# rbuler/multimodal-isic

Measured on AMD Instinct MI355X. Metric: bags/sec (train step) @ 64x224x224 patches/bag, higher is better.
Workload: dtype bf16; 1 GPU; ISIC-shaped attention-MIL: 256 bags x 64x224x224 patches + 128-d radiomics, ResNet-18 encoder, bf16 (BASELINE.json configs[1]); patches_per_bag=64, patch=3x224x224, radiomics_dim=128, parallelism=dp1

## Files before the change

### multimodal-isic_amd/csrc/conv_stem.hip

```cpp
#include <type_traits>

#include "common.h"
#include "slab_sum.inc"
#include "mfma_tile.h"
#include "pool_grad.h"

namespace {

constexpr int TH = 8, TW = 16;
constexpr int PR = 2 * TH + 5, PC = 40;
constexpr int PROW = PC * 8;
constexpr int WROW = 7 * 64 + 16;
constexpr int CPAD = 72;
constexpr int YROW = 128 + 32;
constexpr int STEM_DW_ELEMS = 64 * 7 * 7 * 3;
constexpr int STEM_WGRAD_BLOCKS = 512;
constexpr int STEM_FWD_BLOCKS = 768;

struct StemArgs {
  const unsigned short* in;
  const unsigned short* w;
  unsigned short* out;
  const unsigned short* dy;
  float* dw;
  double* stat_sum;
  double* stat_sumsq;
  int stat_slots;
  int N, Hin, Win, Hout, Wout, tiles_h, tiles_w, total_tiles;
};

constexpr int PATCH_PER_THREAD = (PR * PC + 255) / 256;
__device__ __forceinline__ void fetch_patch(u32x2 (&r)[PATCH_PER_THREAD], const StemArgs& a, int tile, int tid) {
  const int n = tile / (a.tiles_h * a.tiles_w);
  const int t2 = tile - n * (a.tiles_h * a.tiles_w);
  const int oy0 = (t2 / a.tiles_w) * TH, ox0 = (t2 % a.tiles_w) * TW;
#pragma unroll
  for (int u = 0; u < PATCH_PER_THREAD; ++u) {
    const int idx = tid + 256 * u;
    const int pr = idx / PC, pc = idx - pr * PC;
    const int hi = 2 * oy0 - 3 + pr, wi = 2 * ox0 - 3 + pc;
    u32x2 v = {0u, 0u};
    if (tile < a.total_tiles && idx < PR * PC && hi >= 0 && hi < a.Hin && wi >= 0 && wi < a.Win)
      v = *reinterpret_cast<const u32x2*>(a.in + (((size_t)n * a.Hin + hi) * a.Win + wi) * 4);
    r[u] = v;
  }
}
__device__ __forceinline__ void commit_patch(unsigned char* Ps, const u32x2 (&r)[PATCH_PER_THREAD], int tid) {
#pragma unroll
  for (int u = 0; u < PATCH_PER_THREAD; ++u) {
    const int idx = tid + 256 * u;
    if (idx < PR * PC) {
      const int pr = idx / PC, pc = idx - pr * PC;
      *reinterpret_cast<u32x2*>(Ps + pr * PROW + pc * 8) = r[u];
    }
  }
}

__global__ __launch_bounds__(256) void conv_stem_fwd_kernel(StemArgs a) {
  static_assert(TH * TW * CPAD * 2 >= PR * PROW, "the C tile overlays the patch");
  __shared__ __attribute__((aligned(16))) unsigned char smem[64 * WROW + TH * TW * CPAD * 2];
  unsigned char* Ws = smem;
  unsigned char* Ps = smem + 64 * WROW;
  unsigned short* Cs = reinterpret_cast<unsigned short*>(smem + 64 * WROW);
  const int tid = threadIdx.x, lane = tid & 63, wave = tid >> 6;
  const int fi = lane & 15, fg = lane >> 4;

  for (int idx = tid; idx < 64 * 28; idx += 256) {
    const int co = idx / 28, ch = idx - co * 28;
    *reinterpret_cast<u32x4*>(Ws + co * WROW + ch * 16) = *reinterpret_cast<const u32x4*>(a.w + co * 224 + ch * 8);
  }

  u32x2 pre[PATCH_PER_THREAD];
  fetch_patch(pre, a, blockIdx.x, tid);
  float st_s[4][4], st_q[4][4];
#pragma unroll
  for (int j = 0; j < 4; ++j)
#pragma unroll
    for (int r = 0; r < 4; ++r) { st_s[j][r] = 0.f; st_q[j][r] = 0.f; }
  for (int tile = blockIdx.x; tile < a.total_tiles; tile += gridDim.x) {
    const int n = tile / (a.tiles_h * a.tiles_w);
    const int t2 = tile - n * (a.tiles_h * a.tiles_w);
    const int oy0 = (t2 / a.tiles_w) * TH, ox0 = (t2 % a.tiles_w) * TW;
    lds_barrier();
    commit_patch(Ps, pre, tid);
    lds_barrier();
    fetch_patch(pre, a, tile + gridDim.x, tid);

    f32x4 acc[2][4];
#pragma unroll
    for (int i = 0; i < 2; ++i)
#pragma unroll
      for (int j = 0; j < 4; ++j) acc[i][j] = (f32x4){0.f, 0.f, 0.f, 0.f};
#pragma unroll
    for (int kh = 0; kh < 7; ++kh) {
      bf16x8 af[2], bfr[4];
#pragma unroll
      for (int i = 0; i < 2; ++i) {
        const int oyl = wave * 2 + i;
        af[i] = *reinterpret_cast<const bf16x8*>(Ps + (2 * oyl + kh) * PROW + (2 * fi + 2 * fg) * 8);
      }
#pragma unroll
      for (int j = 0; j < 4; ++j)
        bfr[j] = *reinterpret_cast<const bf16x8*>(Ws + (j * 16 + fi) * WROW + kh * 64 + fg * 16);
#pragma unroll
      for (int i = 0; i < 2; ++i)
#pragma unroll
        for (int j = 0; j < 4; ++j)
          acc[i][j] = __builtin_amdgcn_mfma_f32_16x16x32_bf16(bfr[j], af[i], acc[i][j], 0, 0, 0);
    }
    lds_barrier();
#pragma unroll
    for (int i = 0; i < 2; ++i)
#pragma unroll
      for (int j = 0; j < 4; ++j) {
        const int p = (wave * 2 + i) * 16 + fi;
        const u32x2 v = isic_pack_bf16x4(acc[i][j]);
        *reinterpret_cast<u32x2*>(Cs + p * CPAD + j * 16 + fg * 4) = v;
        if (a.stat_sum) {
          const bool in = (oy0 + wave * 2 + i < a.Hout) && (ox0 + fi < a.Wout);
          const float r0 = in ? __uint_as_float(v[0] << 16) : 0.f, r1 = in ? __uint_as_float(v[0] & 0xFFFF0000u) : 0.f;
          const float r2 = in ? __uint_as_float(v[1] << 16) : 0.f, r3 = in ? __uint_as_float(v[1] & 0xFFFF0000u) : 0.f;
          st_s[j][0] += r0; st_q[j][0] += r0 * r0;
          st_s[j][1] += r1; st_q[j][1] += r1 * r1;
          st_s[j][2] += r2; st_q[j][2] += r2 * r2;
          st_s[j][3] += r3; st_q[j][3] += r3 * r3;
        }
      }
    lds_barrier();
    for (int idx = tid; idx < TH * TW * 8; idx += 256) {
      const int p = idx >> 3, ch = idx & 7;
      const int oy = oy0 + (p >> 4), ox = ox0 + (p & 15);
      if (oy < a.Hout && ox < a.Wout)
        __builtin_nontemporal_store(*reinterpret_cast<const u32x4*>(Cs + p * CPAD + ch * 8),
                                    reinterpret_cast<u32x4*>(a.out + (((size_t)n * a.Hout + oy) * a.Wout + ox) * 64 + ch * 8));
    }
  }
  if (a.stat_sum) {
    __shared__ float stat_red[2][4][64];
    lds_barrier();
#pragma unroll
    for (int j = 0; j < 4; ++j)
#pragma unroll
      for (int r = 0; r < 4; ++r) {
        float sv = st_s[j][r], qv = st_q[j][r];
#pragma unroll
        for (int o = 8; o > 0; o >>= 1) { sv += __shfl_xor(sv, o, 16); qv += __shfl_xor(qv, o, 16); }
        if (fi == 0) { stat_red[0][wave][j * 16 + fg * 4 + r] = sv; stat_red[1][wave][j * 16 + fg * 4 + r] = qv; }
      }
    lds_barrier();
    if (tid < 128) {
      const int c = tid & 63, w = tid >> 6;
      const float t = (stat_red[w][0][c] + stat_red[w][1][c]) + (stat_red[w][2][c] + stat_red[w][3][c]);
      const size_t slot = (size_t)(blockIdx.x % a.stat_slots) * 64 + c;
      atomicAdd((w == 0 ? a.stat_sum : a.stat_sumsq) + slot, (double)t);
    }
  }
}

__global__ __launch_bounds__(256) void conv_stem_wgrad_kernel(StemArgs a) {
  __shared__ __attribute__((aligned(16))) unsigned char smem[PR * PROW + TH * TW * YROW];
  unsigned char* Ps = smem;
  unsigned char* Ys = smem + PR * PROW;
  const int tid = threadIdx.x, lane = tid & 63, wave = tid >> 6;
  const int fg = lane >> 4, fi = lane & 15, fq = fi >> 2, fp = fi & 3;
  typedef __attribute__((address_space(3))) s16x4* lds_s16x4;

  f32x4 acc[4][4];
#pragma unroll
  for (int i = 0; i < 4; ++i)
#pragma unroll
    for (int j = 0; j < 4; ++j) acc[i][j] = (f32x4){0.f, 0.f, 0.f, 0.f};

  u32x2 pre[PATCH_PER_THREAD];
  u32x4 prey[4];
  auto fetch_dy = [&](int tile) {
    const int n = tile / (a.tiles_h * a.tiles_w);
    const int t2 = tile - n * (a.tiles_h * a.tiles_w);
    const int oy0 = (t2 / a.tiles_w) * TH, ox0 = (t2 % a.tiles_w) * TW;
#pragma unroll
    for (int u = 0; u < 4; ++u) {
      const int idx = tid + 256 * u;
      const int p = idx >> 3, ch = idx & 7;
      const int oy = oy0 + (p >> 4), ox = ox0 + (p & 15);
      u32x4 v = {0u, 0u, 0u, 0u};
      if (tile < a.total_tiles && oy < a.Hout && ox < a.Wout)
        v = *reinterpret_cast<const u32x4*>(a.dy + (((size_t)n * a.Hout + oy) * a.Wout + ox) * 64 + ch * 8);
      prey[u] = v;
    }
  };
  fetch_patch(pre, a, blockIdx.x, tid);
  fetch_dy(blockIdx.x);
  for (int tile = blockIdx.x; tile < a.total_tiles; tile += gridDim.x) {
    lds_barrier();
    commit_patch(Ps, pre, tid);
#pragma unroll
    for (int u = 0; u < 4; ++u) {
      const int idx = tid + 256 * u;
      *reinterpret_cast<u32x4*>(Ys + (idx >> 3) * YROW + (idx & 7) * 16) = prey[u];
    }
    lds_barrier();
    fetch_patch(pre, a, tile + gridDim.x, tid);
    fetch_dy(tile + gridDim.x);
#pragma unroll
    for (int ks = 0; ks < 4; ++ks) {
      const int k1 = ks * 32 + 8 * fg + fq, k2 = k1 + 4;
      bf16x8 af[4], bfr[4];
#pragma unroll
      for (int i = 0; i < 4; ++i) {
        const s16x4 lo = __builtin_amdgcn_ds_read_tr16_b64_v4i16((lds_s16x4)(Ys + k1 * YROW + (i * 16 + 4 * fp) * 2));
        const s16x4 hi = __builtin_amdgcn_ds_read_tr16_b64_v4i16((lds_s16x4)(Ys + k2 * YROW + (i * 16 + 4 * fp) * 2));
        s16x8_t t; t.lo = lo; t.hi = hi;
        af[i] = __builtin_bit_cast(bf16x8, t);
      }
#pragma unroll
      for (int j = 0; j < 4; ++j) {
        const int nt = wave + 4 * j;
        const int kh = nt >> 1, half = nt & 1;
        const int khc = kh > 6 ? 6 : kh;
        const unsigned char* p1 = Ps + (2 * (k1 >> 4) + khc) * PROW + (2 * (k1 & 15) + half * 4 + fp) * 8;
        const unsigned char* p2 = Ps + (2 * (k2 >> 4) + khc) * PROW + (2 * (k2 & 15) + half * 4 + fp) * 8;
        const s16x4 lo = __builtin_amdgcn_ds_read_tr16_b64_v4i16((lds_s16x4)p1);
        const s16x4 hi = __builtin_amdgcn_ds_read_tr16_b64_v4i16((lds_s16x4)p2);
        s16x8_t t; t.lo = lo; t.hi = hi;
        bfr[j] = __builtin_bit_cast(bf16x8, t);
      }
#pragma unroll
      for (int i = 0; i < 4; ++i)
#pragma unroll
        for (int j = 0; j < 4; ++j)
          acc[i][j] = __builtin_amdgcn_mfma_f32_16x16x32_bf16(af[i], bfr[j], acc[i][j], 0, 0, 0);
    }
  }
#pragma unroll
  for (int i = 0; i < 4; ++i)
#pragma unroll
    for (int j = 0; j < 4; ++j) {
      const int nt = wave + 4 * j;
      if (nt >= 14) continue;
      const int kh = nt >> 1, kw = (nt & 1) * 4 + (fi >> 2), c = fi & 3;
      if (kw >= 7 || c >= 3) continue;
#pragma unroll
      for (int r = 0; r < 4; ++r) {
        const int co = i * 16 + fg * 4 + r;
        a.dw[(size_t)blockIdx.x * STEM_DW_ELEMS + ((co * 7 + kh) * 7 + kw) * 3 + c] = acc[i][j][r];
      }
    }
}

struct StemBnArgs {
  StemArgs s;
  const unsigned short* y0;
  const unsigned char* argmax;
  const unsigned short* gp;
  const float* mean; const float* rstd; const float* gamma; const float* scale; const float* shift;
  const double* dgamma; const double* dbeta;
  float* dgamma_f32; float* dbeta_f32;
  int Hp, Wp;
};

__global__ __launch_bounds__(256, 2) void conv_stem_wgrad_bn_kernel(StemBnArgs b) {
  const StemArgs& a = b.s;
  __shared__ __attribute__((aligned(16))) unsigned char smem[PR * PROW + TH * TW * YROW];
  __shared__ __attribute__((aligned(16))) float cst[5][64];
  unsigned char* Ps = smem;
  unsigned char* Ys = smem + PR * PROW;
  const int tid = threadIdx.x, lane = tid & 63, wave = tid >> 6;
  const int fg = lane >> 4, fi = lane & 15, fq = fi >> 2, fp = fi & 3;
  typedef __attribute__((address_space(3))) s16x4* lds_s16x4;
  const isic_pool::PoolGeom geom{a.Hout, a.Wout, 64, b.Hp, b.Wp};

  if (tid < 64) {
    const float inv_rows = 1.f / (float)((int64_t)a.N * a.Hout * a.Wout);
    const float rs = b.rstd[tid], mu = b.mean[tid], k1 = b.gamma[tid] * rs;
    const float k2 = (float)b.dbeta[tid] * inv_rows, k3 = (float)b.dgamma[tid] * inv_rows;
    cst[0][tid] = k1; cst[1][tid] = -k1 * k3 * rs; cst[2][tid] = k1 * (k3 * rs * mu - k2);
    cst[3][tid] = b.scale[tid]; cst[4][tid] = b.shift[tid];
    if (blockIdx.x == 0 && b.dgamma_f32) {
      b.dgamma_f32[tid] += (float)b.dgamma[tid];
      b.dbeta_f32[tid] += (float)b.dbeta[tid];
    }
  }

  f32x4 acc[4][4];
#pragma unroll
  for (int i = 0; i < 4; ++i)
#pragma unroll
    for (int j = 0; j < 4; ++j) acc[i][j] = (f32x4){0.f, 0.f, 0.f, 0.f};

  const int cg = tid & 7, bl = tid >> 3, al = bl >> 3, bw = bl & 7;
  u32x2 pre[PATCH_PER_THREAD];
  u32x4 xr[4];
  isic_pool::Windows win;
  auto fetch_dy = [&](int tile) {
    const int tc = tile < a.total_tiles ? tile : a.total_tiles - 1;
    const int n = tc / (a.tiles_h * a.tiles_w);
    const int t2 = tc - n * (a.tiles_h * a.tiles_w);
    const int oy0 = (t2 / a.tiles_w) * TH, ox0 = (t2 % a.tiles_w) * TW;
    const int ga = (oy0 >> 1) + al, gb = (ox0 >> 1) + bw;
#pragma unroll
    for (int p = 0; p < 4; ++p) {
      const int hi = min(2 * ga + (p >> 1), a.Hout - 1), wi = min(2 * gb + (p & 1), a.Wout - 1);
      xr[p] = *reinterpret_cast<const u32x4*>(b.y0 + (((size_t)n * a.Hout + hi) * a.Wout + wi) * 64 + cg * 8);
    }
    isic_pool::load_windows(win, b.argmax, b.gp, geom, n, min(ga, b.Hp - 1), min(gb, b.Wp - 1), cg);
  };
  auto commit_dy = [&](int tile) {
    const int n = tile / (a.tiles_h * a.tiles_w);
    const int t2 = tile - n * (a.tiles_h * a.tiles_w);
    const int oy0 = (t2 / a.tiles_w) * TH, ox0 = (t2 % a.tiles_w) * TW;
    const int ga = (oy0 >> 1) + al, gb = (ox0 >> 1) + bw;
    const bool inside = (oy0 + TH <= a.Hout) && (ox0 + TW <= a.Wout);
    auto half = [&](auto HC) {
      constexpr int H_ = decltype(HC)::value;
      float g[4][4];
      isic_pool::windows_to_grad4<H_>(win, geom, ga, gb, g);
      const int c0 = cg * 8 + H_ * 4;
      const f32x4 kA = *reinterpret_cast<const f32x4*>(&cst[0][c0]), kB = *reinterpret_cast<const f32x4*>(&cst[1][c0]);
      const f32x4 kD = *reinterpret_cast<const f32x4*>(&cst[2][c0]), sc = *reinterpret_cast<const f32x4*>(&cst[3][c0]);
      const f32x4 sh = *reinterpret_cast<const f32x4*>(&cst[4][c0]);
#pragma unroll
      for (int p = 0; p < 4; ++p) {
        const int oyl = 2 * al + (p >> 1), oxl = 2 * bw + (p & 1);
        const bool in = inside || ((oy0 + oyl < a.Hout) && (ox0 + oxl < a.Wout));
        const unsigned lo = xr[p][2 * H_], hi = xr[p][2 * H_ + 1];
        float xv[4];
        isic_unpack_bf16x4(lo, hi, xv);
        f32x4 o;
#pragma unroll
        for (int j = 0; j < 4; ++j) {
          const float dz = (xv[j] * sc[j] + sh[j] > 0.f) ? g[p][j] : 0.f;
          o[j] = kA[j] * dz + (kB[j] * xv[j] + kD[j]);
          if (!inside) o[j] = in ? o[j] : 0.f;
        }
        *reinterpret_cast<u32x2*>(Ys + (oyl * TW + oxl) * YROW + cg * 16 + H_ * 8) = isic_pack_bf16x4(o);
      }
    };
    half(std::integral_constant<int, 0>{});
    __builtin_amdgcn_sched_barrier(0);
    half(std::integral_constant<int, 1>{});
  };
  __syncthreads();
  fetch_patch(pre, a, blockIdx.x, tid);
  fetch_dy(blockIdx.x);
  for (int tile = blockIdx.x; tile < a.total_tiles; tile += gridDim.x) {
    lds_barrier();
    commit_patch(Ps, pre, tid);
    commit_dy(tile);
    lds_barrier();
    fetch_patch(pre, a, tile + gridDim.x, tid);
    fetch_dy(tile + gridDim.x);
#pragma unroll
    for (int ks = 0; ks < 4; ++ks) {
      const int k1 = ks * 32 + 8 * fg + fq, k2 = k1 + 4;
      bf16x8 af[4], bfr[4];
#pragma unroll
      for (int i = 0; i < 4; ++i) {
        const s16x4 lo = __builtin_amdgcn_ds_read_tr16_b64_v4i16((lds_s16x4)(Ys + k1 * YROW + (i * 16 + 4 * fp) * 2));
        const s16x4 hi = __builtin_amdgcn_ds_read_tr16_b64_v4i16((lds_s16x4)(Ys + k2 * YROW + (i * 16 + 4 * fp) * 2));
        s16x8_t t; t.lo = lo; t.hi = hi;
        af[i] = __builtin_bit_cast(bf16x8, t);
      }
#pragma unroll
      for (int j = 0; j < 4; ++j) {
        const int nt = wave + 4 * j;
        const int kh = nt >> 1, half = nt & 1;
        const int khc = kh > 6 ? 6 : kh;
        const unsigned char* p1 = Ps + (2 * (k1 >> 4) + khc) * PROW + (2 * (k1 & 15) + half * 4 + fp) * 8;
        const unsigned char* p2 = Ps + (2 * (k2 >> 4) + khc) * PROW + (2 * (k2 & 15) + half * 4 + fp) * 8;
        const s16x4 lo = __builtin_amdgcn_ds_read_tr16_b64_v4i16((lds_s16x4)p1);
        const s16x4 hi = __builtin_amdgcn_ds_read_tr16_b64_v4i16((lds_s16x4)p2);
        s16x8_t t; t.lo = lo; t.hi = hi;
        bfr[j] = __builtin_bit_cast(bf16x8, t);
      }
#pragma unroll
      for (int i = 0; i < 4; ++i)
#pragma unroll
        for (int j = 0; j < 4; ++j)
          acc[i][j] = __builtin_amdgcn_mfma_f32_16x16x32_bf16(af[i], bfr[j], acc[i][j], 0, 0, 0);
    }
  }
#pragma unroll
  for (int i = 0; i < 4; ++i)
#pragma unroll
    for (int j = 0; j < 4; ++j) {
      const int nt = wave + 4 * j;
      if (nt >= 14) continue;
      const int kh = nt >> 1, kw = (nt & 1) * 4 + (fi >> 2), c = fi & 3;
      if (kw >= 7 || c >= 3) continue;
#pragma unroll
      for (int r = 0; r < 4; ++r) {
        const int co = i * 16 + fg * 4 + r;
        a.dw[(size_t)blockIdx.x * STEM_DW_ELEMS + ((co * 7 + kh) * 7 + kw) * 3 + c] = acc[i][j][r];
      }
    }
}

__global__ void stem_pack_kernel(const float* __restrict__ w, unsigned short* __restrict__ ws) {
  const int idx = blockIdx.x * blockDim.x + threadIdx.x;
  if (idx >= 64 * 7 * 8 * 4) return;
  const int c = idx & 3, kw = (idx >> 2) & 7, kh = (idx >> 5) % 7, co = idx / 224;
  float v = 0.f;
  if (c < 3 && kw < 7) v = w[((co * 7 + kh) * 7 + kw) * 3 + c];
  ws[idx] = f32_to_bf16_bits(v);
}

int stem_args(StemArgs& a, int N, int Hin, int Win, int Hout, int Wout) {
  if (Hout != (Hin + 6 - 7) / 2 + 1 || Wout != (Win + 6 - 7) / 2 + 1) return ISIC_ERR_BAD_ARG;
  a.N = N; a.Hin = Hin; a.Win = Win; a.Hout = Hout; a.Wout = Wout;
  a.tiles_h = ceil_div(Hout, TH); a.tiles_w = ceil_div(Wout, TW);
  const int64_t tt = (int64_t)N * a.tiles_h * a.tiles_w;
  if (tt > 0x7FFFFFFFLL) return ISIC_ERR_UNSUPPORTED;
  a.total_tiles = (int)tt;
  return ISIC_OK;
}

}

extern "C" {

int isic_conv_stem_fwd_bf16(const uint16_t* in_nhwc4, const uint16_t* w_stem, uint16_t* out, int N, int Hin, int Win,
                            int Hout, int Wout, void* stream) {
  return isic_conv_stem_fwd_stats_bf16(in_nhwc4, w_stem, out, N, Hin, Win, Hout, Wout, nullptr, nullptr, 0, stream);
}

int isic_conv_stem_fwd_stats_bf16(const uint16_t* in_nhwc4, const uint16_t* w_stem, uint16_t* out, int N, int Hin,
                                  int Win, int Hout, int Wout, double* stat_sum, double* stat_sumsq, int stat_slots,
                                  void* stream) {
  ISIC_CHECK_ARG(in_nhwc4 && w_stem && out && N > 0 && Hin > 0 && Win > 0);
  ISIC_CHECK_ARG((stat_sum == nullptr) == (stat_sumsq == nullptr));
  ISIC_CHECK_ARG(!stat_sum || stat_slots > 0);
  StemArgs a;
  a.stat_sum = stat_sum; a.stat_sumsq = stat_sumsq; a.stat_slots = stat_slots > 0 ? stat_slots : 1;
  a.in = in_nhwc4; a.w = w_stem; a.out = out; a.dy = nullptr; a.dw = nullptr;
  int rc = stem_args(a, N, Hin, Win, Hout, Wout);
  if (rc != ISIC_OK) return rc;
  const int grid = a.total_tiles < STEM_FWD_BLOCKS ? a.total_tiles : STEM_FWD_BLOCKS;
  hipLaunchKernelGGL(conv_stem_fwd_kernel, dim3(grid), dim3(256), 0, as_stream(stream), a);
  return isic_launch_status();
}

size_t isic_conv_stem_wgrad_workspace_bytes(void) { return (size_t)STEM_WGRAD_BLOCKS * STEM_DW_ELEMS * sizeof(float); }

int isic_conv_stem_wgrad_bf16(const uint16_t* in_nhwc4, const uint16_t* dy, float* dw, int N, int Hin, int Win,
                              int Hout, int Wout, void* workspace, size_t workspace_bytes, void* stream) {
  ISIC_CHECK_ARG(in_nhwc4 && dy && dw && workspace && N > 0 && Hin > 0 && Win > 0);
  if (workspace_bytes < isic_conv_stem_wgrad_workspace_bytes()) return ISIC_ERR_WORKSPACE;
  StemArgs a;
  a.stat_sum = nullptr; a.stat_sumsq = nullptr; a.stat_slots = 1;
  a.in = in_nhwc4; a.w = nullptr; a.out = nullptr; a.dy = dy; a.dw = reinterpret_cast<float*>(workspace);
  int rc = stem_args(a, N, Hin, Win, Hout, Wout);
  if (rc != ISIC_OK) return rc;
  const int grid = a.total_tiles < STEM_WGRAD_BLOCKS ? a.total_tiles : STEM_WGRAD_BLOCKS;
  hipLaunchKernelGGL(conv_stem_wgrad_kernel, dim3(grid), dim3(256), 0, as_stream(stream), a);
  isic_slab_reduce_launch(ISIC_SLAB_XOR16, reinterpret_cast<const float*>(workspace), grid, STEM_DW_ELEMS, dw, 1.f,
                          as_stream(stream));
  return isic_launch_status();
}

int isic_conv_stem_wgrad_bn_pooled_bf16(const uint16_t* in_nhwc4, const uint16_t* y0, const uint8_t* argmax,
                                        const uint16_t* dy_pooled, const float* mean, const float* rstd,
                                        const float* gamma, const float* scale, const float* shift, const double* dgamma,
                                        const double* dbeta, float* dw, float* dgamma_f32, float* dbeta_f32, int N,
                                        int Hin, int Win, int Hout, int Wout, int Hp, int Wp, void* workspace,
                                        size_t workspace_bytes, void* stream) {
  ISIC_CHECK_ARG(in_nhwc4 && y0 && argmax && dy_pooled && mean && rstd && gamma && scale && shift && dgamma && dbeta && dw);
  ISIC_CHECK_ARG(workspace != nullptr);
  if (workspace_bytes < isic_conv_stem_wgrad_workspace_bytes()) return ISIC_ERR_WORKSPACE;
  ISIC_CHECK_ARG(N > 0 && Hin > 0 && Win > 0 && (dgamma_f32 == nullptr) == (dbeta_f32 == nullptr));
  ISIC_CHECK_ARG(Hp == (Hout + 2 - 3) / 2 + 1 && Wp == (Wout + 2 - 3) / 2 + 1);
  StemBnArgs b;
  StemArgs& a = b.s;
  a.stat_sum = nullptr; a.stat_sumsq = nullptr; a.stat_slots = 1;
  a.in = in_nhwc4; a.w = nullptr; a.out = nullptr; a.dy = nullptr; a.dw = reinterpret_cast<float*>(workspace);
  int rc = stem_args(a, N, Hin, Win, Hout, Wout);
  if (rc != ISIC_OK) return rc;
  b.y0 = y0; b.argmax = argmax; b.gp = dy_pooled; b.mean = mean; b.rstd = rstd; b.gamma = gamma; b.scale = scale;
  b.shift = shift; b.dgamma = dgamma; b.dbeta = dbeta; b.dgamma_f32 = dgamma_f32; b.dbeta_f32 = dbeta_f32;
  b.Hp = Hp; b.Wp = Wp;
  const int grid = a.total_tiles < STEM_WGRAD_BLOCKS ? a.total_tiles : STEM_WGRAD_BLOCKS;
  hipLaunchKernelGGL(conv_stem_wgrad_bn_kernel, dim3(grid), dim3(256), 0, as_stream(stream), b);
  isic_slab_reduce_launch(ISIC_SLAB_XOR16, reinterpret_cast<const float*>(workspace), grid, STEM_DW_ELEMS, dw, 1.f,
                          as_stream(stream));
  return isic_launch_status();
}

int isic_conv_stem_pack_bf16(const float* w_krsc, uint16_t* w_stem, void* stream) {
  ISIC_CHECK_ARG(w_krsc && w_stem);
  hipLaunchKernelGGL(stem_pack_kernel, dim3(ceil_div(64 * 224, 256)), dim3(256), 0, as_stream(stream), w_krsc, w_stem);
  return isic_launch_status();
}

}
```

Measured before the change: 946.5 bags/s.

## Double-buffer stem wgrad patches via global-to-LDS DMA and specialize interior tiles

```diff
diff --git a/multimodal-isic_amd/csrc/conv_stem.hip b/multimodal-isic_amd/csrc/conv_stem.hip
--- a/multimodal-isic_amd/csrc/conv_stem.hip
+++ b/multimodal-isic_amd/csrc/conv_stem.hip
@@ -258,28 +258,67 @@
   int Hp, Wp;
 };
 
+constexpr int PPIECES = PR * (PROW / 16);
+constexpr int PDMA = (PPIECES + 63) / 64;
+constexpr int PBUF = PDMA * 1024;
+__device__ __attribute__((aligned(256))) unsigned char g_stem_zero_page[256];
+
+struct StemTile { int n, oy0, ox0; };
+
+template <int HALF>
+__device__ __forceinline__ void stem_route4_interior(const isic_pool::Windows& w, float (&out)[4][4]) {
+  float acc[4][4];
+#pragma unroll
+  for (int p = 0; p < 4; ++p)
+#pragma unroll
+    for (int j = 0; j < 4; ++j) acc[p][j] = 0.f;
+#pragma unroll
+  for (int i = 0; i < 2; ++i)
+#pragma unroll
+    for (int jw = 0; jw < 2; ++jw) {
+      const unsigned lo = w.g[i * 2 + jw][2 * HALF], hi = w.g[i * 2 + jw][2 * HALF + 1];
+      const float g[4] = {__uint_as_float(lo << 16), __uint_as_float(lo & 0xFFFF0000u), __uint_as_float(hi << 16),
+                          __uint_as_float(hi & 0xFFFF0000u)};
+      const unsigned am = w.am[i * 2 + jw][HALF];
+#pragma unroll
+      for (int dy = i; dy < 2; ++dy)
+#pragma unroll
+        for (int dx = jw; dx < 2; ++dx) {
+          const unsigned code = (unsigned)((dy + 1 - 2 * i) * 3 + (dx + 1 - 2 * jw));
+#pragma unroll
+          for (int j = 0; j < 4; ++j)
+            if (((am >> (j * 8)) & 0xFFu) == code) acc[dy * 2 + dx][j] += g[j];
+        }
+    }
+#pragma unroll
+  for (int p = 0; p < 4; ++p)
+#pragma unroll
+    for (int j = 0; j < 4; ++j) out[p][j] = bf16_bits_to_f32(f32_to_bf16_bits(acc[p][j]));
+}
+
+__device__ __forceinline__ float stem_dy_unfused(float kA, float kB, float kD, float y0, float dz) {
+#pragma clang fp contract(off)
+  const float t = kD + kB * y0;
+  return t + kA * dz;
+}
+
+template <bool DMA>
 __global__ __launch_bounds__(256, 2) void conv_stem_wgrad_bn_kernel(StemBnArgs b) {
   const StemArgs& a = b.s;
-  __shared__ __attribute__((aligned(16))) unsigned char smem[PR * PROW + TH * TW * YROW];
+  constexpr int PSZ = DMA ? 2 * PBUF : PR * PROW;
+  constexpr int PSH = DMA ? 8 : 0;
+  __shared__ __attribute__((aligned(16))) unsigned char smem[PSZ + TH * TW * YROW];
   __shared__ __attribute__((aligned(16))) float cst[5][64];
-  unsigned char* Ps = smem;
-  unsigned char* Ys = smem + PR * PROW;
-  const int tid = threadIdx.x, lane = tid & 63, wave = tid >> 6;
+  unsigned char* Ys = smem + PSZ;
+  const unsigned lds0 = (unsigned)(size_t)(__attribute__((address_space(3))) unsigned char*)smem;
+  const int tid = threadIdx.x, lane = tid & 63, wave = __builtin_amdgcn_readfirstlane(tid >> 6);
   const int fg = lane >> 4, fi = lane & 15, fq = fi >> 2, fp = fi & 3;
   typedef __attribute__((address_space(3))) s16x4* lds_s16x4;
+  const unsigned frag_y = (unsigned)((8 * fg + fq) * YROW + 8 * fp);
+  const unsigned frag_p = (unsigned)(2 * (fg >> 1) * PROW + (16 * (fg & 1) + 2 * fq + fp) * 8 + PSH);
   const isic_pool::PoolGeom geom{a.Hout, a.Wout, 64, b.Hp, b.Wp};
 
-  if (tid < 64) {
-    const float inv_rows = 1.f / (float)((int64_t)a.N * a.Hout * a.Wout);
-    const float rs = b.rstd[tid], mu = b.mean[tid], k1 = b.gamma[tid] * rs;
-    const float k2 = (float)b.dbeta[tid] * inv_rows, k3 = (float)b.dgamma[tid] * inv_rows;
-    cst[0][tid] = k1; cst[1][tid] = -k1 * k3 * rs; cst[2][tid] = k1 * (k3 * rs * mu - k2);
-    cst[3][tid] = b.scale[tid]; cst[4][tid] = b.shift[tid];
-    if (blockIdx.x == 0 && b.dgamma_f32) {
-      b.dgamma_f32[tid] += (float)b.dgamma[tid];
-      b.dbeta_f32[tid] += (float)b.dbeta[tid];
-    }
-  }
+  const int bid = blockIdx.x;
 
   f32x4 acc[4][4];
 #pragma unroll
@@ -287,33 +326,72 @@
 #pragma unroll
     for (int j = 0; j < 4; ++j) acc[i][j] = (f32x4){0.f, 0.f, 0.f, 0.f};
 
+  const int tiles_img = a.tiles_h * a.tiles_w;
+  const int step_n = (int)gridDim.x / tiles_img, step_r = (int)gridDim.x - step_n * tiles_img;
+  const int step_y = (step_r / a.tiles_w) * TH, step_x = (step_r % a.tiles_w) * TW;
+  const int span_y = a.tiles_h * TH, span_x = a.tiles_w * TW;
+  auto advance = [&](StemTile& t) {
+    t.ox0 += step_x;
+    if (t.ox0 >= span_x) { t.ox0 -= span_x; t.oy0 += TH; }
+    t.oy0 += step_y;
+    if (t.oy0 >= span_y) { t.oy0 -= span_y; t.n += 1; }
+    t.n += step_n;
+  };
+  const bool fits32 = (int64_t)a.Hout * a.Wout < (1 << 24);
+  auto interior = [&](const StemTile& t) { return fits32 && t.oy0 + TH <= a.Hout && t.ox0 + TW <= a.Wout; };
+
   const int cg = tid & 7, bl = tid >> 3, al = bl >> 3, bw = bl & 7;
-  u32x2 pre[PATCH_PER_THREAD];
+  const unsigned yoff = (unsigned)((2 * al * a.Wout + 2 * bw) * 128 + cg * 16);
+  const unsigned goff = (unsigned)((al * b.Wp + bw) * 128 + cg * 16);
+  u32x2 pre[DMA ? 1 : PATCH_PER_THREAD];
   u32x4 xr[4];
   isic_pool::Windows win;
-  auto fetch_dy = [&](int tile) {
-    const int tc = tile < a.total_tiles ? tile : a.total_tiles - 1;
-    const int n = tc / (a.tiles_h * a.tiles_w);
-    const int t2 = tc - n * (a.tiles_h * a.tiles_w);
-    const int oy0 = (t2 / a.tiles_w) * TH, ox0 = (t2 % a.tiles_w) * TW;
-    const int ga = (oy0 >> 1) + al, gb = (ox0 >> 1) + bw;
-#pragma unroll
-    for (int p = 0; p < 4; ++p) {
-      const int hi = min(2 * ga + (p >> 1), a.Hout - 1), wi = min(2 * gb + (p & 1), a.Wout - 1);
-      xr[p] = *reinterpret_cast<const u32x4*>(b.y0 + (((size_t)n * a.Hout + hi) * a.Wout + wi) * 64 + cg * 8);
-    }
-    isic_pool::load_windows(win, b.argmax, b.gp, geom, n, min(ga, b.Hp - 1), min(gb, b.Wp - 1), cg);
+  auto fetch_dy = [&](const StemTile& t, auto INT) {
+    if constexpr (decltype(INT)::value) {
+      const unsigned char* yb = reinterpret_cast<const unsigned char*>(b.y0) +
+                                (((int64_t)t.n * a.Hout + t.oy0) * a.Wout + t.ox0) * 128;
+      const int64_t w0 = ((int64_t)t.n * b.Hp + (t.oy0 >> 1)) * b.Wp + (t.ox0 >> 1);
+      const unsigned char* gb = reinterpret_cast<const unsigned char*>(b.gp) + w0 * 128;
+      const unsigned char* ab = b.argmax + w0 * 64;
+#pragma unroll
+      for (int p = 0; p < 4; ++p)
+        xr[p] = *reinterpret_cast<const u32x4*>(yb + (size_t)(p >> 1) * a.Wout * 128 + yoff + (p & 1) * 128);
+      const unsigned drow = ((t.oy0 >> 1) + al + 1 < b.Hp) ? (unsigned)b.Wp * 128u : 0u;
+      const unsigned dcol = ((t.ox0 >> 1) + bw + 1 < b.Wp) ? 128u : 0u;
+#pragma unroll
+      for (int k = 0; k < 4; ++k) {
+        const unsigned o = goff + ((k >> 1) ? drow : 0u) + ((k & 1) ? dcol : 0u);
+        win.am[k] = *reinterpret_cast<const u32x2*>(ab + (o >> 1));
+        win.g[k] = *reinterpret_cast<const u32x4*>(gb + o);
+      }
+    } else {
+      const int ga = (t.oy0 >> 1) + al, gb = (t.ox0 >> 1) + bw;
+#pragma unroll
+      for (int p = 0; p < 4; ++p) {
+        const int hi = min(2 * ga + (p >> 1), a.Hout - 1), wi = min(2 * gb + (p & 1), a.Wout - 1);
+        xr[p] = *reinterpret_cast<const u32x4*>(b.y0 + (((size_t)t.n * a.Hout + hi) * a.Wout + wi) * 64 + cg * 8);
+      }
+      isic_pool::load_windows(win, b.argmax, b.gp, geom, t.n, min(ga, b.Hp - 1), min(gb, b.Wp - 1), cg);
+    }
   };
-  auto commit_dy = [&](int tile) {
-    const int n = tile / (a.tiles_h * a.tiles_w);
-    const int t2 = tile - n * (a.tiles_h * a.tiles_w);
-    const int oy0 = (t2 / a.tiles_w) * TH, ox0 = (t2 % a.tiles_w) * TW;
-    const int ga = (oy0 >> 1) + al, gb = (ox0 >> 1) + bw;
-    const bool inside = (oy0 + TH <= a.Hout) && (ox0 + TW <= a.Wout);
+  auto commit_dy = [&](const StemTile& t, auto INT) {
+    constexpr bool I_ = decltype(INT)::value;
+    const int ga = (t.oy0 >> 1) + al, gb = (t.ox0 >> 1) + bw;
+    const bool inside = I_ || ((t.oy0 + TH <= a.Hout) && (t.ox0 + TW <= a.Wout));
+    if constexpr (I_) {
+      const bool row1 = ga + 1 < b.Hp, col1 = gb + 1 < b.Wp;
+#pragma unroll
+      for (int k = 1; k < 4; ++k) {
+        const bool live = ((k >> 1) == 0 || row1) && ((k & 1) == 0 || col1);
+        win.am[k][0] = live ? win.am[k][0] : 0xFFFFFFFFu;
+        win.am[k][1] = live ? win.am[k][1] : 0xFFFFFFFFu;
+      }
+    }
     auto half = [&](auto HC) {
       constexpr int H_ = decltype(HC)::value;
       float g[4][4];
-      isic_pool::windows_to_grad4<H_>(win, geom, ga, gb, g);
+      if constexpr (I_) stem_route4_interior<H_>(win, g);
+      else isic_pool::windows_to_grad4<H_>(win, geom, ga, gb, g);
       const int c0 = cg * 8 + H_ * 4;
       const f32x4 kA = *reinterpret_cast<const f32x4*>(&cst[0][c0]), kB = *reinterpret_cast<const f32x4*>(&cst[1][c0]);
       const f32x4 kD = *reinterpret_cast<const f32x4*>(&cst[2][c0]), sc = *reinterpret_cast<const f32x4*>(&cst[3][c0]);
@@ -321,15 +399,15 @@
 #pragma unroll
       for (int p = 0; p < 4; ++p) {
         const int oyl = 2 * al + (p >> 1), oxl = 2 * bw + (p & 1);
-        const bool in = inside || ((oy0 + oyl < a.Hout) && (ox0 + oxl < a.Wout));
+        const bool in = inside || ((t.oy0 + oyl < a.Hout) && (t.ox0 + oxl < a.Wout));
         const unsigned lo = xr[p][2 * H_], hi = xr[p][2 * H_ + 1];
         float xv[4];
         isic_unpack_bf16x4(lo, hi, xv);
         f32x4 o;
 #pragma unroll
         for (int j = 0; j < 4; ++j) {
-          const float dz = (xv[j] * sc[j] + sh[j] > 0.f) ? g[p][j] : 0.f;
-          o[j] = kA[j] * dz + (kB[j] * xv[j] + kD[j]);
+          const float dz = (fmaf(xv[j], sc[j], sh[j]) > 0.f) ? g[p][j] : 0.f;
+          o[j] = stem_dy_unfused(kA[j], kB[j], kD[j], xv[j], dz);
           if (!inside) o[j] = in ? o[j] : 0.f;
         }
         *reinterpret_cast<u32x2*>(Ys + (oyl * TW + oxl) * YROW + cg * 16 + H_ * 8) = isic_pack_bf16x4(o);
@@ -339,36 +417,88 @@
     __builtin_amdgcn_sched_barrier(0);
     half(std::integral_constant<int, 1>{});
   };
+
+  int ppr[2], ppc[2];
+  unsigned poff[2];
+#pragma unroll
+  for (int u = 0; u < 2; ++u) {
+    const int q = (wave + 4 * u) * 64 + lane;
+    ppr[u] = q < PPIECES ? q / (PROW / 16) : -100000;
+    ppc[u] = 2 * (q % (PROW / 16));
+    poff[u] = q < PPIECES ? (unsigned)((ppr[u] * a.Win + ppc[u]) * 8) : 0u;
+  }
+  const unsigned char* zp = g_stem_zero_page + (lane & 7) * 16;
+  auto issue_patch = [&](const StemTile& t, int buf) {
+    const int hi0 = 2 * t.oy0 - 3, wi0 = 2 * t.ox0 - 4;
+    const unsigned char* org = reinterpret_cast<const unsigned char*>(a.in) +
+                               (((int64_t)t.n * a.Hin + hi0) * a.Win + wi0) * 8;
+#pragma unroll
+    for (int u = 0; u < 2; ++u) {
+      const int d = wave + 4 * u;
+      if (d < PDMA) {
+        const bool ok = (unsigned)(hi0 + ppr[u]) < (unsigned)a.Hin && (unsigned)(wi0 + ppc[u]) < (unsigned)a.Win;
+        isic_glds16(ok ? org + poff[u] : zp, __builtin_amdgcn_readfirstlane(lds0 + (unsigned)(buf * PBUF + d * 1024)));
+      }
+    }
+  };
+
+  StemTile cur;
+  {
+    const int t0 = bid;
+    const int n = t0 / tiles_img, t2 = t0 - n * tiles_img;
+    cur.n = n; cur.oy0 = (t2 / a.tiles_w) * TH; cur.ox0 = (t2 % a.tiles_w) * TW;
+  }
+  int buf = 0;
+  if (tid < 64) {
+#pragma clang fp contract(off)
+    const float inv_rows = 1.f / (float)((int64_t)a.N * a.Hout * a.Wout);
+    const float rs = b.rstd[tid], mu = b.mean[tid], k1 = b.gamma[tid] * rs;
+    const float k2 = (float)b.dbeta[tid] * inv_rows, k3 = (float)b.dgamma[tid] * inv_rows;
+    cst[0][tid] = k1;
+    cst[1][tid] = (-k1 * k3) * rs;
+    cst[2][tid] = k1 * fmaf(k3 * rs, mu, -k2);
+    cst[3][tid] = b.scale[tid]; cst[4][tid] = b.shift[tid];
+  }
   __syncthreads();
-  fetch_patch(pre, a, blockIdx.x, tid);
-  fetch_dy(blockIdx.x);
-  for (int tile = blockIdx.x; tile < a.total_tiles; tile += gridDim.x) {
-    lds_barrier();
-    commit_patch(Ps, pre, tid);
-    commit_dy(tile);
-    lds_barrier();
-    fetch_patch(pre, a, tile + gridDim.x, tid);
-    fetch_dy(tile + gridDim.x);
+  if constexpr (DMA) issue_patch(cur, 0);
+  else fetch_patch(pre, a, bid, tid);
+  if (interior(cur)) fetch_dy(cur, std::true_type{});
+  else fetch_dy(cur, std::false_type{});
+  for (int tile = bid; tile < a.total_tiles; tile += gridDim.x) {
+    unsigned char* Ps = smem + (DMA ? buf * PBUF : 0);
+    lds_barrier();
+    if constexpr (!DMA) commit_patch(Ps, pre, tid);
+    if (interior(cur)) commit_dy(cur, std::true_type{});
+    else commit_dy(cur, std::false_type{});
+    if constexpr (DMA) asm volatile("s_waitcnt vmcnt(0)" ::: "memory");
+    lds_barrier();
+    const bool more = tile + (int)gridDim.x < a.total_tiles;
+    if constexpr (!DMA) fetch_patch(pre, a, tile + gridDim.x, tid);
+    if (more) {
+      advance(cur);
+      if constexpr (DMA) issue_patch(cur, buf ^ 1);
+      if (interior(cur)) fetch_dy(cur, std::true_type{});
+      else fetch_dy(cur, std::false_type{});
+    }
+    buf ^= 1;
+    const unsigned char* yb = Ys + frag_y;
+    const unsigned char* pb = Ps + frag_p + ((wave >> 1) * PROW + (wave & 1) * 32);
+    const unsigned char* pb3 = pb - (wave >= 2 ? PROW : 0);
 #pragma unroll
     for (int ks = 0; ks < 4; ++ks) {
-      const int k1 = ks * 32 + 8 * fg + fq, k2 = k1 + 4;
       bf16x8 af[4], bfr[4];
 #pragma unroll
       for (int i = 0; i < 4; ++i) {
-        const s16x4 lo = __builtin_amdgcn_ds_read_tr16_b64_v4i16((lds_s16x4)(Ys + k1 * YROW + (i * 16 + 4 * fp) * 2));
-        const s16x4 hi = __builtin_amdgcn_ds_read_tr16_b64_v4i16((lds_s16x4)(Ys + k2 * YROW + (i * 16 + 4 * fp) * 2));
+        const s16x4 lo = __builtin_amdgcn_ds_read_tr16_b64_v4i16((lds_s16x4)(yb + ks * 32 * YROW + i * 32));
+        const s16x4 hi = __builtin_amdgcn_ds_read_tr16_b64_v4i16((lds_s16x4)(yb + (ks * 32 + 4) * YROW + i * 32));
         s16x8_t t; t.lo = lo; t.hi = hi;
         af[i] = __builtin_bit_cast(bf16x8, t);
       }
 #pragma unroll
       for (int j = 0; j < 4; ++j) {
-        const int nt = wave + 4 * j;
-        const int kh = nt >> 1, half = nt & 1;
-        const int khc = kh > 6 ? 6 : kh;
-        const unsigned char* p1 = Ps + (2 * (k1 >> 4) + khc) * PROW + (2 * (k1 & 15) + half * 4 + fp) * 8;
-        const unsigned char* p2 = Ps + (2 * (k2 >> 4) + khc) * PROW + (2 * (k2 & 15) + half * 4 + fp) * 8;
+        const unsigned char* p1 = (j < 3 ? pb : pb3) + (4 * ks + 2 * j) * PROW;
         const s16x4 lo = __builtin_amdgcn_ds_read_tr16_b64_v4i16((lds_s16x4)p1);
-        const s16x4 hi = __builtin_amdgcn_ds_read_tr16_b64_v4i16((lds_s16x4)p2);
+        const s16x4 hi = __builtin_amdgcn_ds_read_tr16_b64_v4i16((lds_s16x4)(p1 + 64));
         s16x8_t t; t.lo = lo; t.hi = hi;
         bfr[j] = __builtin_bit_cast(bf16x8, t);
       }
@@ -390,9 +520,13 @@
 #pragma unroll
       for (int r = 0; r < 4; ++r) {
         const int co = i * 16 + fg * 4 + r;
-        a.dw[(size_t)blockIdx.x * STEM_DW_ELEMS + ((co * 7 + kh) * 7 + kw) * 3 + c] = acc[i][j][r];
-      }
-    }
+        a.dw[(size_t)bid * STEM_DW_ELEMS + ((co * 7 + kh) * 7 + kw) * 3 + c] = acc[i][j][r];
+      }
+    }
+  if (bid == 0 && tid < 64 && b.dgamma_f32) {
+    b.dgamma_f32[tid] += (float)b.dgamma[tid];
+    b.dbeta_f32[tid] += (float)b.dbeta[tid];
+  }
 }
 
 __global__ void stem_pack_kernel(const float* __restrict__ w, unsigned short* __restrict__ ws) {
@@ -478,7 +612,10 @@
   b.shift = shift; b.dgamma = dgamma; b.dbeta = dbeta; b.dgamma_f32 = dgamma_f32; b.dbeta_f32 = dbeta_f32;
   b.Hp = Hp; b.Wp = Wp;
   const int grid = a.total_tiles < STEM_WGRAD_BLOCKS ? a.total_tiles : STEM_WGRAD_BLOCKS;
-  hipLaunchKernelGGL(conv_stem_wgrad_bn_kernel, dim3(grid), dim3(256), 0, as_stream(stream), b);
+  if (Win % 2 == 0 && (reinterpret_cast<uintptr_t>(in_nhwc4) & 15) == 0)
+    hipLaunchKernelGGL(conv_stem_wgrad_bn_kernel<true>, dim3(grid), dim3(256), 0, as_stream(stream), b);
+  else
+    hipLaunchKernelGGL(conv_stem_wgrad_bn_kernel<false>, dim3(grid), dim3(256), 0, as_stream(stream), b);
   isic_slab_reduce_launch(ISIC_SLAB_XOR16, reinterpret_cast<const float*>(workspace), grid, STEM_DW_ELEMS, dw, 1.f,
                           as_stream(stream));
   return isic_launch_status();
```

Result: faster. 964.9 bags/s (median of 6 runs) (+1.9%).
